# intel/neural-speed

Hardware: AMD Instinct MI355X
Metric: decode_tokens_per_sec (higher is better)
Workload: dtype f16; 1 GPU; Llama-2-7B Q4_0 (BesTLA int4 sym g32 bf16-scale) batch=1 decode GEMM chain: 32 layers x {QKV, WO, FFN gate/up, FFN down} + lm_head; parallelism=tp1, launch=hipGraph replay, weights_bytes_per_gpu=3716481024

## Files before the change

neural-speed_amd/csrc/ns_gemv.hip:

```cpp
#include <hip/hip_runtime.h>

#include <algorithm>
#include <atomic>
#include <cmath>
#include <cstddef>
#include <cstdlib>
#include <cstring>
#include <type_traits>
#include <utility>

#include "../../include/ns_bestla.h"
#include "ns_common.h"
#include "ns_route.h"
#include "ns_dev.h"

namespace ns {

#ifndef NS_GV_PF
#define NS_GV_PF 4
#endif
constexpr int kGvPF = NS_GV_PF;
constexpr int kGvMaxRows = 16;
constexpr size_t kGvMaxALds = 64 * 1024;
constexpr size_t kGvMaxLds = 160 * 1024;
// ... 66 lines not shown
  GemvRope rope;
  F4Lut lut;
  F8Consts f8;
#ifdef NS_TRACE
  unsigned long long* trace;
#endif
};
using KArgs = const __attribute__((address_space(4))) GemvParams*;
__device__ __forceinline__ KArgs late_args() {
  uint64_t v = reinterpret_cast<uint64_t>(__builtin_amdgcn_kernarg_segment_ptr());
  asm volatile("" : "+s"(v));
  return reinterpret_cast<KArgs>(v);
}

#ifdef NS_TRACE
#define NS_GSTAMP(i)                                                                                     \
  do {                                                                                                   \
    __builtin_amdgcn_sched_barrier(0);                                                                   \
    if ((threadIdx.x & 63) == 0 && blockIdx.x < 4096)                                                     \
      p.trace[(size_t(blockIdx.x) * 16 + (threadIdx.x >> 6)) * 8 + (i)] = wall_clock64();                 \
    __builtin_amdgcn_sched_barrier(0);                                                                   \
  } while (0)
#else
#define NS_GSTAMP(i)
#endif

template <int N>
__device__ __forceinline__ void wait_vmcnt() {
  asm volatile("s_waitcnt vmcnt(%0)" ::"n"(N) : "memory");
}

enum GemvMode { GV_PLAIN = 0, GV_DUAL = 1, GV_MSEG = 2 };
constexpr int kGvA32Regs = 8;
template <int KIND, int SPS, int SK, bool ASYM, int MODE, int XV, bool PL = false>
__global__ __launch_bounds__(1024) void gemv_kernel(const GemvParams p) {
  constexpr bool EXT = XV == 1, MOE = XV == 4, I8Q = XV == 5, A32 = XV == 2 || MOE || I8Q, I8S = XV == 3 || I8Q;
  static_assert(!PL || ((KIND == WK_INT4 || KIND == WK_INT8) && !I8S && !MOE), "native planes: integer formats, fp16 numerics");
  static_assert(!I8S || KIND == WK_INT4 || KIND == WK_INT8, "integer weights only");
  constexpr uint32_t AEL = I8S ? 1u : 2u;
  constexpr bool DUAL = MODE == GV_DUAL, MSEG = MODE == GV_MSEG;
  constexpr int NJ = kind_is_8bit(KIND) ? 2 : 4;
  constexpr int KSTEP = NJ * 32;
  constexpr int NQ = DUAL ? 2 : 1;
  constexpr int PF = kGvPF;
  static_assert(PF % NQ == 0, "ring slots alternate between the two matrices");
  constexpr int SBYTES = SPS * (SK == SK_F32 ? 4 : 2);
  using Corr = CorrRaw<SPS, SK, ASYM>;
  extern __shared__ __attribute__((aligned(16))) unsigned char smem[];
  _Float16* a_lds = reinterpret_cast<_Float16*>(smem);
  NS_GSTAMP(0);

  {
    asm volatile("" ::"s"(p.wbase0), "s"(p.a), "s"(p.ks), "s"(p.qstride), "s"(p.nw_log2), "s"(p.s_off0), "s"(p.sstride),
                 "s"(p.srows), "s"(p.srow_mul), "s"(p.srow_shift), "s"(p.m), "s"(p.k), "s"(p.lda), "s"(p.row_stride),
                 "s"(p.ring_off), "s"(p.ring_stride));
    if constexpr (DUAL) asm volatile("" ::"s"(p.wbase1), "s"(p.s_off1));
    if constexpr (MSEG)
      asm volatile("" ::"s"(p.tb1), "s"(p.tb2), "s"(p.mat[0].wbase), "s"(p.mat[1].wbase), "s"(p.mat[2].wbase), "s"(p.mat[0].s_off),
                   "s"(p.mat[1].s_off), "s"(p.mat[2].s_off));
    if constexpr (ASYM) asm volatile("" ::"s"(p.z_off0), "s"(p.z_off1), "s"(p.zstride));
    if constexpr (PL) asm volatile("" ::"s"(p.pl_bits), "s"(p.pl_lanes));
  }
  const int tid = threadIdx.x;
  const uint32_t w = __builtin_amdgcn_readfirstlane(tid >> 6);
  const int l = tid & 63;
  const int nn = l & 15, g = l >> 4;
  const uint32_t NW = 1u << p.nw_log2;
  const uint32_t ks = p.ks;
  const uint32_t T = blockIdx.x;
// ... 20 lines not shown
    const int e = *p.moe_id;
    if (e < 0 || e >= p.moe_n) {
      const KArgs cz = late_args();
      const int colz = int(T) * 16 + nn;
      if (w == 0 && g == 0 && colz < cz->mat[0].n) {
        float v = 0.f;
        const float dv = cz->d ? cz->d[colz] : 0.f;
        switch (cz->epilogue) {
          case 1: v = v + dv; break;
          case 2: v = v * dv; break;
          case 3: v = epi_gelu(v + dv); break;
          case 4: v = epi_gelu(v); break;
          case 5: v = epi_silu(v); break;
          default: break;
        }
        cz->mat[0].c[colz] = v;
        if (cz->mat[0].c16) cz->mat[0].c16[colz] = (_Float16)v;
      }
      return;
    }
    rw[0] = make_rsrc(p.moe_table[e].codes, 0x80000000u);
    so[0] = p.s_off0;
    zo[0] = p.z_off0;
  } else {
    rw[0] = make_rsrc(p.wbase0, 0x80000000u);
    so[0] = p.s_off0;
    zo[0] = p.z_off0;
  }
  const uint32_t tile_q = tl * ks * p.qstride;
  const uint32_t tile_c = tl * p.srows;
  const uint32_t voff_q = l * 16, voff_s = nn * SBYTES, voff_z = nn * SPS;
  const I4Consts i4c = {0x000f000fu, 0x00f000f0u, 0x64006400u};

  constexpr uint32_t SLOT = 1024u + 16u * SBYTES + (ASYM ? 16u * SPS : 0u);
  constexpr int OPS = ASYM ? 3 : 2;
  static_assert(OPS * PF + kGvMaxRows * 2 <= 63, "vmcnt is a 6-bit counter (ring + the carried norm's pieces)");
  const LdsPtr ring = (LdsPtr)(smem) + p.ring_off + w * p.ring_stride;
  const uint32_t ring_lane = uint32_t(reinterpret_cast<uintptr_t>(ring)) + uint32_t(l) * 16u;
  const uint32_t ring_corr = uint32_t(reinterpret_cast<uintptr_t>(ring)) + 1024u + uint32_t(nn) * SBYTES;

  auto issue = [&](auto slot_c, uint32_t s) {
    constexpr int slot = decltype(slot_c)::value;
    constexpr int q = slot % NQ;
#if defined(__HIP_DEVICE_COMPILE__)
    const uint32_t crow = tile_c + ((s * p.srow_mul) >> p.srow_shift);
    const LdsPtr dst = ring + slot * SLOT;
    if (!PL || uint32_t(l) < p.pl_lanes)
      __builtin_amdgcn_raw_ptr_buffer_load_lds(rw[q], reinterpret_cast<__attribute__((address_space(3))) void*>(dst), 16, voff_q,
                                               tile_q + s * p.qstride, 0, 2);
    if (l < SBYTES)
      __builtin_amdgcn_raw_ptr_buffer_load_lds(rw[q], reinterpret_cast<__attribute__((address_space(3))) void*>(dst + 1024), 16,
                                               voff_q, so[q] + crow * p.sstride, 0, 2);
    if constexpr (ASYM) {
      if (l < SPS)
        __builtin_amdgcn_raw_ptr_buffer_load_lds(rw[q], reinterpret_cast<__attribute__((address_space(3))) void*>(dst + 1024 + 16 * SBYTES),
                                                 16, voff_q, zo[q] + crow * p.zstride, 0, 2);
    }
#endif
  };
  auto wait_records = [&](uint32_t younger) {
    if (younger == uint32_t(PF - 1)) {
      wait_vmcnt<OPS * (PF - 1)>();
      return;
    }
    [&]<int... K>(std::integer_sequence<int, K...>) {
      (void)((younger == uint32_t(K) ? (wait_vmcnt<OPS * K>(), true) : false) || ...);
    }(std::make_integer_sequence<int, PF + 1>{});
  };

#define NS_FOR_SLOTS(BODY)                                        \
  {                                                               \
    [&]<int... I>(std::integer_sequence<int, I...>) {             \
      (([&] { constexpr int i = I; std::integral_constant<int, I> ic; (void)i; (void)ic; BODY }()), ...); \
    }(std::make_integer_sequence<int, PF>{});                     \
  }

  const int rows = min(p.m, kGvMaxRows);
  floatx4 areg[A32 ? kGvA32Regs : 1];
  if constexpr (A32) {
    const uint64_t abase = reinterpret_cast<uint64_t>(p.a);
    const uint4v ra_words = {uint32_t(abase), uint32_t(abase >> 32) & 0xffffu,
                             uint32_t(rows - 1) * uint32_t(p.lda) * 4u + uint32_t(p.k) * 4u, 0x00020000u};
    const uint32_t row_bytes = ks * uint32_t(KSTEP) * 4u;
    const uint32_t pieces = (row_bytes + 1023u) >> 10;
    const uint32_t total = uint32_t(rows) * pieces;
    uint32_t r = 0, c = w;
#pragma unroll
    for (int i = 0; i < kGvA32Regs; i++) {
      const uint32_t u = w + (uint32_t(i) << p.nw_log2);
      areg[i] = floatx4{0.f, 0.f, 0.f, 0.f};
      if (u < total) {
// ... 10 lines not shown
  } else {
    const Rsrc ra = make_rsrc(p.a, uint32_t(rows - 1) * uint32_t(p.lda) * AEL + uint32_t(p.k) * AEL);
    const uint32_t row_bytes = ks * uint32_t(KSTEP) * AEL;
    const uint32_t pieces = (row_bytes + 1023u) >> 10;
    const uint32_t total = uint32_t(rows) * pieces;
    const LdsPtr al = (LdsPtr)(smem);
    for (uint32_t u = w; u < total; u += NW) {
      uint32_t r = 0, c = u;
      if (rows > 1) {
        r = u / pieces;
        c = u - r * pieces;
      }
      const uint32_t left = row_bytes - (c << 10);
#if defined(__HIP_DEVICE_COMPILE__)
      if (uint32_t(l) * 16u < left)
        __builtin_amdgcn_raw_ptr_buffer_load_lds(ra, reinterpret_cast<__attribute__((address_space(3))) void*>(al + r * p.row_stride * 2u + (c << 10)),
                                                 16, voff_q, r * uint32_t(p.lda) * AEL + (c << 10), 0, 0);
#endif
    }
    if constexpr (I8S) {
      const Rsrc rc = make_rsrc(p.i8_corr, p.i8_span);
      for (uint32_t u = w; u < ((p.i8_span + 1023u) >> 10); u += NW) {
#if defined(__HIP_DEVICE_COMPILE__)
        __builtin_amdgcn_raw_ptr_buffer_load_lds(rc, reinterpret_cast<__attribute__((address_space(3))) void*>(al + p.ssq_off + (u << 10)), 16,
                                                 voff_q, u << 10, 0, 0);
#endif
      }
    }
  }
  __builtin_amdgcn_sched_barrier(0);

  const uint32_t first = w;
  const uint32_t nst = first < ks ? (ks - first + NW - 1) >> p.nw_log2 : 0u;
  NS_FOR_SLOTS({ if (uint32_t(i / NQ) < nst) issue(ic, first + ((i / NQ) << p.nw_log2)); })
  __builtin_amdgcn_sched_barrier(0);
  NS_GSTAMP(1);

  const float* in_ssq = nullptr;
  uint32_t in_parts = 0, ssq_off = 0;
  if constexpr (EXT) {
    const KArgs mid = late_args();
    in_ssq = mid->in_ssq;
    in_parts = mid->in_parts;
    ssq_off = mid->ssq_off;
  }
  if (EXT && in_ssq && w == 0) {
    const uint32_t in_stride = late_args()->in_stride;
    const uint32_t spieces = (in_parts * 4u + 1023u) >> 10;
    const Rsrc rs = make_rsrc(in_ssq, (uint32_t(rows - 1) * in_stride + in_parts) * 4u);
    const LdsPtr al = (LdsPtr)(smem);
    for (uint32_t u = 0; u < uint32_t(rows) * spieces; u++) {
      const uint32_t r = u / spieces, c = u - r * spieces;
      const uint32_t left = in_parts * 4u - (c << 10);
#if defined(__HIP_DEVICE_COMPILE__)
      if (uint32_t(l) * 16u < left)
        __builtin_amdgcn_raw_ptr_buffer_load_lds(rs, reinterpret_cast<__attribute__((address_space(3))) void*>(al + ssq_off + (u << 10)),
                                                 16, voff_q, r * in_stride * 4u + (c << 10), 0, 0);
#endif
    }
  }
  __builtin_amdgcn_sched_barrier(0);

  wait_records(min(nst * uint32_t(NQ), uint32_t(PF)));
  if constexpr (A32) {
#pragma unroll
    for (int i = 0; i < kGvA32Regs; i++) asm volatile("" : "+v"(areg[i]));
    const uint32_t row_bytes = ks * uint32_t(KSTEP) * 4u;
    const uint32_t pieces = (row_bytes + 1023u) >> 10;
    const uint32_t total = uint32_t(rows) * pieces;
    uint32_t r = 0, c = w;
    if constexpr (I8Q) {
      const uint32_t lds0q = uint32_t(reinterpret_cast<uintptr_t>((LdsPtr)(smem)));
      const uint32_t lpb = 1u << (p.i8_bshift - 2u);
      const uint32_t k_bytes = uint32_t(p.k) * 4u;
#pragma unroll
      for (int i = 0; i < kGvA32Regs; i++) {
        const uint32_t u = w + (uint32_t(i) << p.nw_log2);
        if (u < total) {
          while (c >= pieces) c -= pieces, r++;
          const floatx4 v = areg[i];
          float maxval = 1.17549435e-38f , minval = 0.f;
#pragma unroll
          for (int e = 0; e < 4; e++) {
            maxval = v[e] > maxval ? v[e] : maxval;
            minval = v[e] < minval ? v[e] : minval;
          }
          auto dpp = [](float x, auto ctrl) {
            return __builtin_bit_cast(float, __builtin_amdgcn_update_dpp(0, __builtin_bit_cast(int, x), decltype(ctrl)::value, 0xf, 0xf, false));
          };
          auto combine = [&](float om, float on) {
            maxval = om > maxval ? om : maxval;
            minval = on < minval ? on : minval;
          };
          combine(dpp(maxval, std::integral_constant<int, 0xB1>{}), dpp(minval, std::integral_constant<int, 0xB1>{}));
          combine(dpp(maxval, std::integral_constant<int, 0x4E>{}), dpp(minval, std::integral_constant<int, 0x4E>{}));
          combine(dpp(maxval, std::integral_constant<int, 0x141>{}), dpp(minval, std::integral_constant<int, 0x141>{}));
// ... 25 lines not shown
        }
      }
    } else {
#pragma unroll
    for (int i = 0; i < kGvA32Regs; i++) {
      const uint32_t u = w + (uint32_t(i) << p.nw_log2);
      if (u < total) {
        while (c >= pieces) c -= pieces, r++;
        const half2_t lo = half2_t{(_Float16)areg[i][0], (_Float16)areg[i][1]};
        const half2_t hi = half2_t{(_Float16)areg[i][2], (_Float16)areg[i][3]};
        const uint32_t dst = uint32_t(reinterpret_cast<uintptr_t>((LdsPtr)(smem))) + r * p.row_stride * 2u + (c << 9) + uint32_t(l) * 8u;
        if ((c << 10) + uint32_t(l) * 16u < row_bytes)
          asm volatile("ds_write_b64 %0, %1" ::"v"(dst), "v"((uint64_t(as_u32(hi)) << 32) | as_u32(lo)) : "memory");
        c += NW;
      }
    }
    }
    asm volatile("s_waitcnt lgkmcnt(0)" ::: "memory");
  }
  asm volatile("s_barrier" ::: "memory");
  NS_GSTAMP(2);

  const uint32_t aoff = uint32_t(min(nn, rows - 1)) * p.row_stride + 8 * g;
  floatx4 acc[NQ];
#pragma unroll
  for (int q = 0; q < NQ; q++) acc[q] = floatx4{0.f, 0.f, 0.f, 0.f};

  float accr[NQ][4];
#pragma unroll
  for (int q = 0; q < NQ; q++)
#pragma unroll
    for (int r = 0; r < 4; r++) accr[q][r] = 0.f;
  const uint32_t i8_rsb = p.row_stride * 2u;
  auto compute = [&](auto slot_c, uint32_t s) {
    constexpr int slot = decltype(slot_c)::value;
    constexpr int q = slot % NQ;
#if defined(NS_GV_ABL) && NS_GV_ABL == 1
    (void)s;
    return;
#endif
    if constexpr (I8S) {
      Corr cr;
      {
        typedef __attribute__((address_space(3))) const uint32_t* L32;
        const uint32_t ca = ring_corr + uint32_t(slot) * SLOT;
        if constexpr (SBYTES == 2) {
          cr.s[0] = *reinterpret_cast<__attribute__((address_space(3))) const uint16_t*>(ca);
        } else {
#pragma unroll
          for (int t = 0; t < Corr::NW32; t++) cr.s[t] = reinterpret_cast<L32>(ca)[t];
        }
        if constexpr (ASYM) {
          const uint32_t za = uint32_t(reinterpret_cast<uintptr_t>(ring)) + uint32_t(slot) * SLOT + 1024u + 16u * SBYTES + uint32_t(nn) * SPS;
          if constexpr (SPS == 4)
            cr.z[0] = *reinterpret_cast<L32>(za);
          else if constexpr (SPS == 2)
            cr.z[0] = *reinterpret_cast<__attribute__((address_space(3))) const uint16_t*>(za);
          else
            cr.z[0] = *reinterpret_cast<__attribute__((address_space(3))) const uint8_t*>(za);
        }
      }
      float sc[4], zp[4];
      corr_decode<SPS, SK, ASYM, NJ>(cr, sc, zp);
      const uint4v qvv = *reinterpret_cast<const __attribute__((address_space(3))) uint4v*>(ring_lane + uint32_t(slot) * SLOT);
      const uint32_t xw[4] = {qvv.x, qvv.y, qvv.z, qvv.w};
      constexpr int BIAS = KIND == WK_INT4 ? 8 : 128;
      const uint32_t lds0 = uint32_t(reinterpret_cast<uintptr_t>((LdsPtr)(smem)));
      const uint32_t kbase = s * uint32_t(KSTEP);
      const uint32_t i8_sbase = lds0 + p.ssq_off;
// ... 27 lines not shown
                "ds_read_b32 %8, %17\n\tds_read_b32 %9, %18\n\tds_read_b32 %10, %19\n\tds_read_b32 %11, %20\n\ts_waitcnt lgkmcnt(0)"
                : "=&v"(av[0]), "=&v"(av[1]), "=&v"(av[2]), "=&v"(av[3]), "=&v"(zau[0]), "=&v"(zau[1]), "=&v"(zau[2]), "=&v"(zau[3]),
                  "=&v"(asu[0]), "=&v"(asu[1]), "=&v"(asu[2]), "=&v"(asu[3])
                : "v"(aaddr), "v"(zrow + kb[0]), "v"(zrow + kb[1]), "v"(zrow + kb[2]), "v"(zrow + kb[3]), "v"(srow + kb[0] * 4u),
                  "v"(srow + kb[1] * 4u), "v"(srow + kb[2] * 4u), "v"(srow + kb[3] * 4u)
                : "memory");
          } else {
            asm volatile(
                "ds_read_b64 %0, %6\n\tds_read_b64 %1, %6 offset:32\n\tds_read_u8 %2, %7\n\tds_read_u8 %3, %8\n\t"
                "ds_read_b32 %4, %9\n\tds_read_b32 %5, %10\n\ts_waitcnt lgkmcnt(0)"
                : "=&v"(av[0]), "=&v"(av[1]), "=&v"(zau[0]), "=&v"(zau[1]), "=&v"(asu[0]), "=&v"(asu[1])
                : "v"(aaddr), "v"(zrow + kb[0]), "v"(zrow + kb[1]), "v"(srow + kb[0] * 4u), "v"(srow + kb[1] * 4u)
                : "memory");
          }
#pragma unroll
          for (int j = 0; j < NJ; j++) {
            if (kbase + 32u * uint32_t(j) < uint32_t(p.k)) {
              const uint32_t avx = uint32_t(av[j]), avy = uint32_t(av[j] >> 32);
              const int za = int(zau[j]);
              const int dot = int(__builtin_amdgcn_udot4(avx, u0[j], __builtin_amdgcn_udot4(avy, u1[j], 0u, false), false));
              const int sa = int(__builtin_amdgcn_udot4(avx, 0x01010101u, __builtin_amdgcn_udot4(avy, 0x01010101u, 0u, false), false));
              const int isum = dot - zbq[j] * sa - za * su[j] + 8 * za * zbq[j];
              accr[q][r] += float(isum) * (__builtin_bit_cast(float, asu[j]) * sc[j]);
            }
          }
        }
      }
      return;
    }
    const _Float16* abase = a_lds + s * KSTEP + aoff;
    Corr cr;
    {
      typedef __attribute__((address_space(3))) const uint32_t* L32;
      const uint32_t ca = ring_corr + uint32_t(slot) * SLOT;
      if constexpr (SBYTES == 2) {
        cr.s[0] = *reinterpret_cast<__attribute__((address_space(3))) const uint16_t*>(ca);
      } else {
#pragma unroll
        for (int t = 0; t < Corr::NW32; t++) cr.s[t] = reinterpret_cast<L32>(ca)[t];
      }
      if constexpr (ASYM) {
        const uint32_t za = uint32_t(reinterpret_cast<uintptr_t>(ring)) + uint32_t(slot) * SLOT + 1024u + 16u * SBYTES + uint32_t(nn) * SPS;
        if constexpr (SPS == 4)
          cr.z[0] = *reinterpret_cast<L32>(za);
        else if constexpr (SPS == 2)
          cr.z[0] = *reinterpret_cast<__attribute__((address_space(3))) const uint16_t*>(za);
        else
          cr.z[0] = *reinterpret_cast<__attribute__((address_space(3))) const uint8_t*>(za);
      }
    }
    float sc[4], zp[4];
    corr_decode<SPS, SK, ASYM, NJ>(cr, sc, zp);
    uint32_t xw[4];
    if constexpr (!PL) {
      const uint4v qvv = *reinterpret_cast<const __attribute__((address_space(3))) uint4v*>(ring_lane + uint32_t(slot) * SLOT);
      xw[0] = qvv.x, xw[1] = qvv.y, xw[2] = qvv.z, xw[3] = qvv.w;
    } else {
      typedef const __attribute__((address_space(3))) uint32_t* L32;
      typedef const __attribute__((address_space(3))) uint16_t* L16;
      typedef uint32_t uint2v __attribute__((ext_vector_type(2)));
      const uint32_t rec = uint32_t(reinterpret_cast<uintptr_t>(ring)) + uint32_t(slot) * SLOT;
      const uint32_t bits = p.pl_bits;
      if constexpr (KIND == WK_INT4) {
        uint32_t a0 = 0, a1 = 0, cw = 0;
        if (bits >= 2) {
          const uint2v av = *reinterpret_cast<const __attribute__((address_space(3))) uint2v*>(rec + 8u * uint32_t(l));
          a0 = av.x, a1 = av.y;
// ... 28 lines not shown
        bq[j] = cvt_i4x8(xw[j], i4c, half2_t{zl, zl}, half2_t{zh, zh});
      } else if constexpr (KIND == WK_INT8) {
        if constexpr (PL) {
          const _Float16 zo8 = (_Float16)(-1024.f - full - zp[j]);
          bq[j] = cvt_u8x8(xw[2 * j], xw[2 * j + 1], half2_t{zo8, zo8});
        } else {
          const _Float16 zo8 = (_Float16)(-1152.f - zp[j]);
          bq[j] = cvt_i8x8(xw[2 * j], xw[2 * j + 1], half2_t{zo8, zo8});
        }
      } else if constexpr (KIND == WK_F8) {
        bq[j] = cvt_f8x8(xw[2 * j], xw[2 * j + 1], p.f8);
      } else {
        bq[j] = cvt_f4x8(xw[j], p.lut);
      }
    }
    floatx4 dd[NJ];
#pragma unroll
    for (int j = 0; j < NJ; j++) {
      const half8_t afrag = *reinterpret_cast<const half8_t*>(abase + 32 * j);
      dd[j] = __builtin_amdgcn_mfma_f32_16x16x32_f16(afrag, bq[j], floatx4{0.f, 0.f, 0.f, 0.f}, 0, 0, 0);
    }
#pragma unroll
    for (int j = 0; j < NJ; j++) acc[q] += dd[j] * sc[j];
  };

  constexpr int SPR = PF / NQ;
  const uint32_t rounds = (nst + SPR - 1) / SPR;
  const uint32_t nitems = nst * NQ;
  for (uint32_t r = 0; r < rounds; r++) {
    NS_FOR_SLOTS({
      const uint32_t ord = r * SPR + i / NQ;
      if (ord < nst) {
        const uint32_t t = r * PF + i;
        wait_records(min(nitems - t - 1, uint32_t(PF - 1)));
        compute(ic, first + (ord << p.nw_log2));
        __builtin_amdgcn_sched_barrier(0);
        if (ord + SPR < nst) issue(ic, first + ((ord + SPR) << p.nw_log2));
        __builtin_amdgcn_sched_barrier(0);
      }
    })
  }
  NS_GSTAMP(4);

  if constexpr (I8S) {
#pragma unroll
    for (int q = 0; q < NQ; q++) {
      float t[4];
#pragma unroll
      for (int r = 0; r < 4; r++) {
        float v = accr[q][r];
        v += __shfl_xor(v, 16, 64);
        v += __shfl_xor(v, 32, 64);
        t[r] = v;
      }
      acc[q] = g == 0 ? floatx4{t[0], t[1], t[2], t[3]} : floatx4{0.f, 0.f, 0.f, 0.f};
    }
  }
  floatx4* red = reinterpret_cast<floatx4*>(smem + p.ring_off);
  const uint32_t kRedWave = p.ring_stride / 16;
#pragma unroll
  for (int q = 0; q < NQ; q++) red[w * kRedWave + q * 64 + l] = acc[q];
  const KArgs cold = late_args();
  const auto* mp = &cold->mat[MSEG ? sg : 0];
  const int ncols = mp->n;
  float* cbase = mp->c;
  _Float16* c16 = mp->c16;
  const int ldc = cold->ldc, ldd = cold->ldd, epi = cold->epilogue;
  const float* dptr = cold->d;
  float* c2 = cold->c2;
// ... 108 lines not shown
            case 5: v = epi_silu(v); break;
            default: break;
          }
        }
        cbase[size_t(row) * ldc + col] = v;
        if (c16) c16[size_t(row) * ldc + col] = (_Float16)(v * gam);
        if constexpr (EXT) {
          if (ogamma && fabsf(v * gam) > 65504.f && cold->out_ovf) __hip_atomic_store(cold->out_ovf, 1u, __ATOMIC_RELAXED, __HIP_MEMORY_SCOPE_SYSTEM);
        }
      }
      if (EXT && ossq) {
        float t = ok ? v * v : 0.f;
        t += __shfl_xor(t, 1, 64);
        t += __shfl_xor(t, 2, 64);
        t += __shfl_xor(t, 4, 64);
        t += __shfl_xor(t, 8, 64);
        if (nn == 0 && row < p.m) ossq[size_t(row) * ostride + tl] = t;
      }
    }
  }
#undef NS_FOR_SLOTS
  NS_GSTAMP(6);
#ifdef NS_TRACE
  if ((threadIdx.x & 63) == 0 && blockIdx.x < 4096)
    p.trace[(size_t(blockIdx.x) * 16 + (threadIdx.x >> 6)) * 8 + 7] =
        (uint64_t(__builtin_amdgcn_s_getreg((31 << 11) | 20)) << 32) | uint32_t(__builtin_amdgcn_s_getreg((31 << 11) | 4));
#endif
}

constexpr int kGvModeA32 = 0x100;
constexpr int kGvModeI8 = 0x200;
constexpr int kGvModeMoe = 0x400;
constexpr int kGvModePlanes = 0x800;
template <int KIND, int SPS, int SK, bool ASYM>
static hipError_t launch_gemv_planes(const GemvParams& p, int mode, int grid, int nw, size_t lds, hipStream_t st) {
  if constexpr ((KIND == WK_INT4 || KIND == WK_INT8) && SK != SK_F16) {
    const dim3 g(grid), b(nw * 64);
    const bool ext = p.in_ssq || p.out_gamma || p.out_ssq || p.rope.on;
    const bool a32 = (mode & kGvModeA32) != 0;
    mode &= 3;
#define NS_GVP(MODEV, EXTV)                                                                                                  \
  {                                                                                                                         \
    auto k = gemv_kernel<KIND, SPS, SK, ASYM, MODEV, EXTV, true>;                                                            \
    static const hipError_t attr =                                                                                          \
        hipFuncSetAttribute(reinterpret_cast<const void*>(k), hipFuncAttributeMaxDynamicSharedMemorySize, int(kGvMaxLds));   \
    if (attr != hipSuccess && lds > 64 * 1024) return attr;                                                                 \
    hipLaunchKernelGGL(k, g, b, lds, st, p);                                                                                \
  }
#define NS_GVP_M(MODEV)                                                              \
  {                                                                                 \
    if (ext) NS_GVP(MODEV, 1) else if (a32) NS_GVP(MODEV, 2) else NS_GVP(MODEV, 0)   \
  }
    if (mode == GV_DUAL)
      NS_GVP_M(GV_DUAL)
    else if (mode == GV_MSEG)
      NS_GVP_M(GV_MSEG)
    else
      NS_GVP_M(GV_PLAIN)
#undef NS_GVP_M
#undef NS_GVP
    return hipGetLastError();
  } else {
    return hipErrorNotSupported;
  }
}
template <int KIND, int SPS, int SK, bool ASYM>
static hipError_t launch_gemv_k(const GemvParams& p, int mode, int grid, int nw, size_t lds, hipStream_t st) {
  if (mode & kGvModePlanes) return launch_gemv_planes<KIND, SPS, SK, ASYM>(p, mode & ~kGvModePlanes, grid, nw, lds, st);
  const dim3 g(grid), b(nw * 64);
  const bool ext = p.in_ssq || p.out_gamma || p.out_ssq || p.rope.on;
  const bool a32 = (mode & kGvModeA32) != 0;
  const bool i8s = (mode & kGvModeI8) != 0;
  const bool moe = (mode & kGvModeMoe) != 0;
  mode &= ~(kGvModeA32 | kGvModeI8 | kGvModeMoe);
  if (moe) {
    if constexpr (KIND == WK_F8) return hipErrorNotSupported;
    if (mode != GV_PLAIN) return hipErrorNotSupported;
  }
  if constexpr (KIND != WK_INT4 && KIND != WK_INT8)
    if (i8s) return hipErrorNotSupported;
#define NS_GV_LAUNCH(MODEV)                                                                                     \
  {                                                                                                             \
    if (moe) NS_GV_LAUNCH_MOE(MODEV) else if (ext) NS_GV_LAUNCH_E(MODEV, 1) else if (i8s && a32) NS_GV_LAUNCH_I8Q(MODEV) else if (a32) NS_GV_LAUNCH_E(MODEV, 2) else if (i8s) NS_GV_LAUNCH_I8(MODEV)    \
    else NS_GV_LAUNCH_E(MODEV, 0)                                                                               \
  }
#define NS_GV_LAUNCH_MOE(MODEV)                                                                                  \
  {                                                                                                             \
    if constexpr (KIND != WK_F8 && MODEV == GV_PLAIN) NS_GV_LAUNCH_E(GV_PLAIN, 4)                               \
  }
#define NS_GV_LAUNCH_I8Q(MODEV)                                                                                  \
  {                                                                                                             \
    if constexpr (KIND == WK_INT4 || KIND == WK_INT8) NS_GV_LAUNCH_E(MODEV, 5)                                  \
  }
#define NS_GV_LAUNCH_I8(MODEV)                                                                                   \
  {                                                                                                             \
    if constexpr (KIND == WK_INT4 || KIND == WK_INT8) NS_GV_LAUNCH_E(MODEV, 3)                                  \
  }
#define NS_GV_LAUNCH_E(MODEV, EXTV)                                                                             \
  {                                                                                                             \
    auto k = gemv_kernel<KIND, SPS, SK, ASYM, MODEV, EXTV>;                                                      \
    static const hipError_t attr =                                                                              \
        hipFuncSetAttribute(reinterpret_cast<const void*>(k), hipFuncAttributeMaxDynamicSharedMemorySize, int(kGvMaxLds)); \
    if (attr != hipSuccess && lds > 64 * 1024) return attr;                                                     \
    hipLaunchKernelGGL(k, g, b, lds, st, p);                                                                    \
  }
  if (mode == GV_DUAL)
    NS_GV_LAUNCH(GV_DUAL)
  else if (mode == GV_MSEG)
    NS_GV_LAUNCH(GV_MSEG)
  else
    NS_GV_LAUNCH(GV_PLAIN)
#undef NS_GV_LAUNCH
#undef NS_GV_LAUNCH_E
#undef NS_GV_LAUNCH_I8
#undef NS_GV_LAUNCH_I8Q
#undef NS_GV_LAUNCH_MOE
  return hipGetLastError();
}
template <int KIND, int SPS, int SK>
static hipError_t launch_gemv_a(const GemvParams& p, bool asym, int mode, int grid, int nw, size_t lds,
                                hipStream_t st) {
  if constexpr (KIND == WK_F4 || KIND == WK_F8) {
    (void)asym;
    return launch_gemv_k<KIND, SPS, SK, false>(p, mode, grid, nw, lds, st);
  } else {
    if (asym) return launch_gemv_k<KIND, SPS, SK, true>(p, mode, grid, nw, lds, st);
    return launch_gemv_k<KIND, SPS, SK, false>(p, mode, grid, nw, lds, st);
  }
}
template <int KIND, int SPS>
static hipError_t launch_gemv_s(const GemvParams& p, uint32_t scale_dt, bool asym, int mode, int grid, int nw,
                                size_t lds, hipStream_t st) {
  if (scale_dt == DT_F32) return launch_gemv_a<KIND, SPS, SK_F32>(p, asym, mode, grid, nw, lds, st);
  if (scale_dt == DT_F16) return launch_gemv_a<KIND, SPS, SK_F16>(p, asym, mode, grid, nw, lds, st);
  return launch_gemv_a<KIND, SPS, SK_BF16>(p, asym, mode, grid, nw, lds, st);
}

#ifdef NS_TRACE
unsigned long long* trace_buffer();
#endif

static std::atomic<int> g_gemv_mode{-1};
void set_gemv_mode(int mode) { g_gemv_mode.store(mode); }
static int gemv_mode() {
  int m = g_gemv_mode.load();
  if (m < 0) {
// ... 2 lines not shown
    g_gemv_mode.store(m);
  }
  return m;
}

static std::atomic<int> g_decode_waves{0};
void set_decode_waves(int nw) { g_decode_waves.store(nw); }
int decode_waves(int grid, int ks, bool dual) {
  int nw = (grid <= 320 && ks >= 32 && ks <= 48 && !dual) ? 16 : 8;
  if (dual) {
    nw = grid * 4 >= 1300 ? 4 : 8;
  } else {
    const int target_waves = 2560;
    while (nw > 2 && grid * (nw / 2) >= target_waves) nw /= 2;
  }
  static const int env_nw0 = getenv("NS_GV_NW") ? atoi(getenv("NS_GV_NW")) : 0;
  const int forced = g_decode_waves.load();
  const int env_nw = forced ? forced : env_nw0;
  if (env_nw == 2 || env_nw == 4 || env_nw == 8 || (env_nw == 16 && !dual)) nw = env_nw;
  while (nw > 1 && nw > ks) nw /= 2;
  return nw;
}

static std::atomic<int> g_gemv_planes{-1};
void set_gemv_planes(int on) { g_gemv_planes.store(on != 0); }
static bool gemv_planes() {
  int v = g_gemv_planes.load();
  if (v < 0) {
    const char* e = getenv("NS_GEMV_PLANES");
    v = e ? atoi(e) != 0 : 1;
    g_gemv_planes.store(v);
  }
  return v != 0;
}

hipError_t launch_gemv(const SmallMArgs& a, hipStream_t st) {
  if (gemv_mode() == 0 || a.m < 1 || a.m > kGvMaxRows) return hipErrorNotSupported;
  const int nmat = a.nseg;
  bool planes = gemv_planes() && !a.i8 && !a.moe;
  for (int i = 0; i < nmat; i++)
    planes = planes && a.seg[i].w->native && a.seg[i].w->native->scale_dt != DT_F16 && a.seg[i].w->native->pl_bits == a.seg[0].w->native->pl_bits;
  auto pick = [&](const ns_weight* w) { return planes ? static_cast<const ns_weight*>(w->native) : w; };
  const ns_weight* w0 = pick(a.seg[0].w);
  GemvParams p;
  memset(&p, 0, sizeof(p));
  uint32_t tiles = 0;
  uint32_t tbeg[3] = {0, 0xffffffffu, 0xffffffffu};
  const uint8_t* wb[3] = {nullptr, nullptr, nullptr};
  uint32_t soff[3] = {0, 0, 0}, zoff[3] = {0, 0, 0};
  for (int i = 0; i < nmat; i++) {
    const ns_weight* w = pick(a.seg[i].w);
    if (!w->single_span || w->alloc_bytes >= (size_t(1) << 31)) return hipErrorNotSupported;
    wb[i] = reinterpret_cast<const uint8_t*>(w->codes);
    soff[i] = uint32_t(reinterpret_cast<const uint8_t*>(w->scales) - wb[i]);
    zoff[i] = w->zps ? uint32_t(reinterpret_cast<const uint8_t*>(w->zps) - wb[i]) : 0u;
    tbeg[i] = a.dual ? 0u : tiles;
    if (!a.dual || i == 0) tiles += uint32_t(w->ntiles);
    p.mat[i] = GemvMat{wb[i], soff[i], zoff[i], tbeg[i], w->n, a.seg[i].c, static_cast<_Float16*>(a.seg[i].c16)};
  }
  const bool mseg = !a.dual && nmat > 1;
  const int mode = a.dual ? GV_DUAL : (mseg ? GV_MSEG : GV_PLAIN);
  p.wbase0 = wb[0];
  p.wbase1 = wb[1];
  p.s_off0 = soff[0], p.s_off1 = soff[1], p.z_off0 = zoff[0], p.z_off1 = zoff[1];
  p.tb1 = mseg ? tbeg[1] : 0xffffffffu;
  p.tb2 = (mseg && nmat > 2) ? tbeg[2] : 0xffffffffu;
// ... 52 lines not shown
    if (k.out_ssq || k.out_gamma) {
      if (a.dual || nmat != 1 || (k.out_ssq && k.out_stride < w0->ntiles)) return hipErrorInvalidValue;
      p.out_gamma = k.out_gamma, p.out_ssq = k.out_ssq, p.out_stride = uint32_t(k.out_stride);
      p.out_ovf = k.out_gamma ? kvm_overflow_word() : nullptr;
    }
  }
  if (a.rope) {
    const ns_qkv_rope& r = *a.rope;
    if (mode != GV_MSEG || nmat != 3 || r.mode != 0 || r.head_size < 2 || (r.head_size & 1) || r.n_dims != r.head_size ||
        !r.kcache16 || !r.vcache16 || !r.cos_sin || r.n_past < 0 || p.mat[0].n != r.heads * r.head_size ||
        p.mat[1].n != r.heads_kv * r.head_size || p.mat[2].n != r.heads_kv * r.head_size)
      return hipErrorInvalidValue;
    p.rope.kc = static_cast<_Float16*>(r.kcache16), p.rope.vc = static_cast<_Float16*>(r.vcache16);
    p.rope.c_sl = r.cache_step_sl, p.rope.c_head = r.cache_step_head;
    p.rope.head_size = r.head_size, p.rope.n_past = r.n_past;
    p.rope.cos_sin = reinterpret_cast<const float2*>(r.cos_sin);
    p.rope.on = 1;
    if (a.rope_route) {
      const QkvRopeRoute& q = *a.rope_route;
      if (rows != 1) return hipErrorInvalidValue;
      p.rope.kmove = q.kmove, p.rope.kd_pos = q.kd_pos;
      p.rope.k32 = q.k32, p.rope.v32 = q.v32;
      p.rope.k32_head = q.k32_head, p.rope.k32_dim = q.k32_dim, p.rope.k32_tok = q.k32_tok;
      p.rope.v32_head = q.v32_head, p.rope.v32_dim = q.v32_dim, p.rope.v32_tok = q.v32_tok;
      p.rope.ovf = q.overflow;
    }
  }
  if (uint64_t(rows) * uint64_t(a.lda) * 4 >= (uint64_t(1) << 30)) return hipErrorNotSupported;

  const int grid = int(tiles);
  const int nq = a.dual ? 2 : 1;
  const uint32_t sbytes = uint32_t(w0->sps) * (w0->scale_dt == DT_F32 ? 4u : 2u);
  const uint32_t slot = 1024u + 16u * sbytes + (w0->asym ? 16u * uint32_t(w0->sps) : 0u);
  auto ring_bytes = [&](int waves) {
    const uint32_t items = ((ks + uint32_t(waves) - 1) / uint32_t(waves)) * uint32_t(nq);
    const size_t b = size_t(std::min<uint32_t>(items, uint32_t(kGvPF))) * slot;
    return std::max<size_t>((b + 15) & ~size_t(15), size_t(nq) * 1024);
  };
  int nw = decode_waves(grid, int(ks), a.dual);
  {
    while (nw > 1 && ((a_bytes + 15) & ~size_t(15)) + ssq_bytes + size_t(nw) * ring_bytes(nw) > kGvMaxLds) nw /= 2;
  }
  uint32_t nw_log2 = 0;
  while ((1 << nw_log2) < nw) nw_log2++;
  if (a32 && uint64_t(rows) * ((uint64_t(ks) * uint32_t(kstep) * 4u + 1023u) >> 10) > uint64_t(nw) * kGvA32Regs) {
    if (i8q) return a.i8->quantized ? hipErrorNotSupported : hipErrorNotReady;
    return hipErrorNotSupported;
  }

  p.ks = ks;
  p.qstride = w0->qstride;
  p.nw_log2 = nw_log2;
  p.sstride = w0->sstride;
  p.zstride = w0->zstride;
  p.srows = uint32_t(w0->srows);
  {
    int mul, shift;
    if (!srow_params(w0, &mul, &shift)) return hipErrorNotSupported;
    p.srow_mul = uint32_t(mul), p.srow_shift = uint32_t(shift);
  }
  p.m = a.m;
  p.k = w0->k;
  p.lda = i8q ? a.i8->lda32 : i8s ? a.i8->ldq : a.lda;
  p.row_stride = row_stride;
  p.ssq_off = uint32_t((a_bytes + 15) & ~size_t(15));
  p.ring_off = p.ssq_off + uint32_t(ssq_bytes);
  p.c2 = a.c2;
  p.d = a.d;
  p.ldc = a.ldc;
  p.ldd = a.ldd;
  p.epilogue = a.epilogue;
  if (w0->kind == WK_F4) f4_lut_planes(w0->lut, &p.lut);
  p.f8 = f8_consts(w0->qtype);
#ifdef NS_TRACE
  p.trace = trace_buffer();
#endif
  p.ring_stride = uint32_t(ring_bytes(nw));
  const size_t lds = size_t(p.ring_off) + size_t(nw) * p.ring_stride;
  if (lds > kGvMaxLds) return hipErrorNotSupported;
  if (moe) {
    p.moe_table = static_cast<const MoeExpertRow*>(a.moe->table);
    p.moe_id = a.moe->id;
    p.moe_n = a.moe->n_as;
  }
  p.pl_bits = planes ? uint32_t(w0->pl_bits) : 0u;
  p.pl_lanes = planes ? w0->code_rec / 16u : 64u;
  const int mode_x = mode | (a32 && !moe ? kGvModeA32 : 0) | (i8s ? kGvModeI8 : 0) | (moe ? kGvModeMoe : 0) | (planes ? kGvModePlanes : 0);

#define NS_DISPATCH(KIND)                                                                       \
  switch (w0->sps) {                                                                            \
    case 4: return launch_gemv_s<KIND, 4>(p, w0->scale_dt, w0->asym, mode_x, grid, nw, lds, st);  \
    case 2: return launch_gemv_s<KIND, 2>(p, w0->scale_dt, w0->asym, mode_x, grid, nw, lds, st);  \
    default: return launch_gemv_s<KIND, 1>(p, w0->scale_dt, w0->asym, mode_x, grid, nw, lds, st); \
  }
  if (w0->kind == WK_INT4) {
    NS_DISPATCH(WK_INT4)
  } else if (w0->kind == WK_INT8) {
    if (w0->sps == 2) return launch_gemv_s<WK_INT8, 2>(p, w0->scale_dt, w0->asym, mode_x, grid, nw, lds, st);
    return launch_gemv_s<WK_INT8, 1>(p, w0->scale_dt, w0->asym, mode_x, grid, nw, lds, st);
  } else if (w0->kind == WK_F8) {
    if (w0->sps == 2) return launch_gemv_a<WK_F8, 2, SK_F32>(p, false, mode_x, grid, nw, lds, st);
    return launch_gemv_a<WK_F8, 1, SK_F32>(p, false, mode_x, grid, nw, lds, st);
  } else {
    NS_DISPATCH(WK_F4)
  }
#undef NS_DISPATCH
}

void touch_gemv_module() {
  hipFuncAttributes fa;
  (void)hipFuncGetAttributes(&fa, reinterpret_cast<const void*>(gemv_kernel<WK_INT4, 4, SK_BF16, false, GV_PLAIN, 0>));
  (void)hipGetLastError();
}
}
```

Baseline: 939.7 tokens/s.

## Gather bf16 group scales for four k-steps in one batched LDS load

For the int4 sym g32 bf16-scale path, the per-slot 16-lane scale buffer load is dropped. Each wave instead issues one gathered load that fetches the scales for four upcoming k-steps into a small double-buffered LDS region, and the vmcnt accounting is rewritten to match. This cuts the number of tiny global loads and vmcnt slots per k-step, and shrinks each ring slot. The cost is extra waits, an lgkmcnt drain before each gather, and more complex, error-prone counter bookkeeping. A host check keeps the path off unless alignment, bounds and LDS-occupancy conditions hold, and an environment variable can disable it.

```diff
diff --git a/neural-speed_amd/csrc/ns_gemv.hip b/neural-speed_amd/csrc/ns_gemv.hip
--- a/neural-speed_amd/csrc/ns_gemv.hip
+++ b/neural-speed_amd/csrc/ns_gemv.hip
@@ -122,9 +122,11 @@
 
 enum GemvMode { GV_PLAIN = 0, GV_DUAL = 1, GV_MSEG = 2 };
 constexpr int kGvA32Regs = 8;
-template <int KIND, int SPS, int SK, bool ASYM, int MODE, int XV, bool PL = false>
+template <int KIND, int SPS, int SK, bool ASYM, int MODE, int XV, bool PL = false, bool SG = false>
 __global__ __launch_bounds__(1024) void gemv_kernel(const GemvParams p) {
   constexpr bool EXT = XV == 1, MOE = XV == 4, I8Q = XV == 5, A32 = XV == 2 || MOE || I8Q, I8S = XV == 3 || I8Q;
+  static_assert(!SG || (KIND == WK_INT4 && SPS == 4 && SK == SK_BF16 && !ASYM && !PL && MODE != GV_DUAL && (XV == 0 || XV == 1) && kGvPF == 4),
+                "scale gather: the flagship's instantiations only");
   static_assert(!PL || ((KIND == WK_INT4 || KIND == WK_INT8) && !I8S && !MOE), "native planes: integer formats, fp16 numerics");
   static_assert(!I8S || KIND == WK_INT4 || KIND == WK_INT8, "integer weights only");
   constexpr uint32_t AEL = I8S ? 1u : 2u;
@@ -211,9 +213,10 @@
   const uint32_t voff_q = l * 16, voff_s = nn * SBYTES, voff_z = nn * SPS;
   const I4Consts i4c = {0x000f000fu, 0x00f000f0u, 0x64006400u};
 
-  constexpr uint32_t SLOT = 1024u + 16u * SBYTES + (ASYM ? 16u * SPS : 0u);
-  constexpr int OPS = ASYM ? 3 : 2;
-  static_assert(OPS * PF + kGvMaxRows * 2 <= 63, "vmcnt is a 6-bit counter (ring + the carried norm's pieces)");
+  constexpr uint32_t SLOT = SG ? 1024u : 1024u + 16u * SBYTES + (ASYM ? 16u * SPS : 0u);
+  constexpr int OPS = SG ? 1 : (ASYM ? 3 : 2);
+  constexpr int GIF = SG ? 2 : 0;
+  static_assert(OPS * PF + GIF + kGvMaxRows * 2 <= 63, "vmcnt is a 6-bit counter (ring + gathers + the carried norm's pieces)");
   const LdsPtr ring = (LdsPtr)(smem) + p.ring_off + w * p.ring_stride;
   const uint32_t ring_lane = uint32_t(reinterpret_cast<uintptr_t>(ring)) + uint32_t(l) * 16u;
   const uint32_t ring_corr = uint32_t(reinterpret_cast<uintptr_t>(ring)) + 1024u + uint32_t(nn) * SBYTES;
@@ -222,11 +225,12 @@
     constexpr int slot = decltype(slot_c)::value;
     constexpr int q = slot % NQ;
 #if defined(__HIP_DEVICE_COMPILE__)
-    const uint32_t crow = tile_c + ((s * p.srow_mul) >> p.srow_shift);
+    const uint32_t crow = SG ? 0u : tile_c + ((s * p.srow_mul) >> p.srow_shift);
     const LdsPtr dst = ring + slot * SLOT;
     if (!PL || uint32_t(l) < p.pl_lanes)
       __builtin_amdgcn_raw_ptr_buffer_load_lds(rw[q], reinterpret_cast<__attribute__((address_space(3))) void*>(dst), 16, voff_q,
                                                tile_q + s * p.qstride, 0, 2);
+    if constexpr (SG) return;
     if (l < SBYTES)
       __builtin_amdgcn_raw_ptr_buffer_load_lds(rw[q], reinterpret_cast<__attribute__((address_space(3))) void*>(dst + 1024), 16,
                                                voff_q, so[q] + crow * p.sstride, 0, 2);
@@ -236,6 +240,11 @@
                                                  16, voff_q, zo[q] + crow * p.zstride, 0, 2);
     }
 #endif
+  };
+  auto wait_requests = [&](uint32_t n) {
+    [&]<int... K>(std::integer_sequence<int, K...>) {
+      (void)((n == uint32_t(K) ? (wait_vmcnt<K>(), true) : false) || ...);
+    }(std::integer_sequence<int, 4, 3, 2, 1, 0, 5, 6>{});
   };
   auto wait_records = [&](uint32_t younger) {
     if (younger == uint32_t(PF - 1)) {
@@ -312,6 +321,24 @@
 
   const uint32_t first = w;
   const uint32_t nst = first < ks ? (ks - first + NW - 1) >> p.nw_log2 : 0u;
+  const LdsPtr sring = ring + p.ring_stride - 1024u;
+  const uint32_t sring_corr = uint32_t(reinterpret_cast<uintptr_t>(sring)) + uint32_t(nn) * SBYTES;
+  const uint32_t voff_g = SG ? ((uint32_t(l) >> 3) << p.nw_log2) * p.sstride + (uint32_t(l) & 7u) * 16u : 0u;
+  (void)sring_corr;
+  (void)voff_g;
+  auto gather = [&](uint32_t j) {
+#if defined(__HIP_DEVICE_COMPILE__)
+    if (uint32_t(l) < 32u && 4u * j + (uint32_t(l) >> 3) < nst)
+      __builtin_amdgcn_raw_ptr_buffer_load_lds(rw[0], reinterpret_cast<__attribute__((address_space(3))) void*>(sring + (j & 1u) * 512u), 16,
+                                               voff_g, so[0] + (tile_c + first + ((4u * j) << p.nw_log2)) * p.sstride, 0, 2);
+#endif
+  };
+  (void)gather;
+  (void)wait_requests;
+  if constexpr (SG) {
+    if (nst > 0u) gather(0u);
+    if (nst > 4u) gather(1u);
+  }
   NS_FOR_SLOTS({ if (uint32_t(i / NQ) < nst) issue(ic, first + ((i / NQ) << p.nw_log2)); })
   __builtin_amdgcn_sched_barrier(0);
   NS_GSTAMP(1);
@@ -341,7 +368,8 @@
   }
   __builtin_amdgcn_sched_barrier(0);
 
-  wait_records(min(nst * uint32_t(NQ), uint32_t(PF)));
+  if constexpr (SG) wait_requests(min(nst, uint32_t(PF)) + (nst > 0u ? 1u : 0u) + (nst > 4u ? 1u : 0u));
+  else wait_records(min(nst * uint32_t(NQ), uint32_t(PF)));
   if constexpr (A32) {
 #pragma unroll
     for (int i = 0; i < kGvA32Regs; i++) asm volatile("" : "+v"(areg[i]));
@@ -433,9 +461,10 @@
 #pragma unroll
     for (int r = 0; r < 4; r++) accr[q][r] = 0.f;
   const uint32_t i8_rsb = p.row_stride * 2u;
-  auto compute = [&](auto slot_c, uint32_t s) {
+  auto compute = [&](auto slot_c, uint32_t s, uint32_t ord) {
     constexpr int slot = decltype(slot_c)::value;
     constexpr int q = slot % NQ;
+    (void)ord;
 #if defined(NS_GV_ABL) && NS_GV_ABL == 1
     (void)s;
     return;
@@ -529,7 +558,7 @@
     Corr cr;
     {
       typedef __attribute__((address_space(3))) const uint32_t* L32;
-      const uint32_t ca = ring_corr + uint32_t(slot) * SLOT;
+      const uint32_t ca = SG ? sring_corr + (ord & 7u) * 128u : ring_corr + uint32_t(slot) * SLOT;
       if constexpr (SBYTES == 2) {
         cr.s[0] = *reinterpret_cast<__attribute__((address_space(3))) const uint16_t*>(ca);
       } else {
@@ -624,9 +653,20 @@
       const uint32_t ord = r * SPR + i / NQ;
       if (ord < nst) {
         const uint32_t t = r * PF + i;
-        wait_records(min(nitems - t - 1, uint32_t(PF - 1)));
-        compute(ic, first + (ord << p.nw_log2));
+        if constexpr (SG) {
+          const uint32_t gathers = (i != PF - 1 && r > 0u && 4u * r + 4u < nst) ? 1u : 0u;
+          wait_requests(min(nst - t - 1, uint32_t(PF - 1)) + gathers);
+        } else {
+          wait_records(min(nitems - t - 1, uint32_t(PF - 1)));
+        }
+        compute(ic, first + (ord << p.nw_log2), ord);
         __builtin_amdgcn_sched_barrier(0);
+        if constexpr (SG) {
+          if (i == PF - 1 && 4u * r + 8u < nst) {
+            asm volatile("s_waitcnt lgkmcnt(0)" ::: "memory");
+            gather(r + 2u);
+          }
+        }
         if (ord + SPR < nst) issue(ic, first + ((ord + SPR) << p.nw_log2));
         __builtin_amdgcn_sched_barrier(0);
       }
@@ -801,6 +841,9 @@
 constexpr int kGvModeI8 = 0x200;
 constexpr int kGvModeMoe = 0x400;
 constexpr int kGvModePlanes = 0x800;
+constexpr int kGvModeSG = 0x1000;
+template <int KIND, int SPS, int SK, bool ASYM, int MODE, int XV>
+constexpr bool kGvHasSG = KIND == WK_INT4 && SPS == 4 && SK == SK_BF16 && !ASYM && MODE != GV_DUAL && (XV == 0 || XV == 1) && kGvPF == 4;
 template <int KIND, int SPS, int SK, bool ASYM>
 static hipError_t launch_gemv_planes(const GemvParams& p, int mode, int grid, int nw, size_t lds, hipStream_t st) {
   if constexpr ((KIND == WK_INT4 || KIND == WK_INT8) && SK != SK_F16) {
@@ -841,7 +884,8 @@
   const bool a32 = (mode & kGvModeA32) != 0;
   const bool i8s = (mode & kGvModeI8) != 0;
   const bool moe = (mode & kGvModeMoe) != 0;
-  mode &= ~(kGvModeA32 | kGvModeI8 | kGvModeMoe);
+  const bool sg = (mode & kGvModeSG) != 0;
+  mode &= ~(kGvModeA32 | kGvModeI8 | kGvModeMoe | kGvModeSG);
   if (moe) {
     if constexpr (KIND == WK_F8) return hipErrorNotSupported;
     if (mode != GV_PLAIN) return hipErrorNotSupported;
@@ -867,7 +911,14 @@
   }
 #define NS_GV_LAUNCH_E(MODEV, EXTV)                                                                             \
   {                                                                                                             \
-    auto k = gemv_kernel<KIND, SPS, SK, ASYM, MODEV, EXTV>;                                                      \
+    if (sg) {                                                                                                   \
+      if constexpr (kGvHasSG<KIND, SPS, SK, ASYM, MODEV, EXTV>) NS_GV_LAUNCH_K(MODEV, EXTV, true)               \
+      else return hipErrorInvalidValue;            \
+    } else NS_GV_LAUNCH_K(MODEV, EXTV, false)                                                                   \
+  }
+#define NS_GV_LAUNCH_K(MODEV, EXTV, SGV)                                                                        \
+  {                                                                                                             \
+    auto k = gemv_kernel<KIND, SPS, SK, ASYM, MODEV, EXTV, false, SGV>;                                          \
     static const hipError_t attr =                                                                              \
         hipFuncSetAttribute(reinterpret_cast<const void*>(k), hipFuncAttributeMaxDynamicSharedMemorySize, int(kGvMaxLds)); \
     if (attr != hipSuccess && lds > 64 * 1024) return attr;                                                     \
@@ -881,6 +932,7 @@
     NS_GV_LAUNCH(GV_PLAIN)
 #undef NS_GV_LAUNCH
 #undef NS_GV_LAUNCH_E
+#undef NS_GV_LAUNCH_K
 #undef NS_GV_LAUNCH_I8
 #undef NS_GV_LAUNCH_I8Q
 #undef NS_GV_LAUNCH_MOE
@@ -949,6 +1001,23 @@
     g_gemv_planes.store(v);
   }
   return v != 0;
+}
+
+static bool device_lds_and_cus(int dev, size_t* lds, int* cus) {
+  constexpr int kMaxDev = 64;
+  static std::atomic<int> s_lds[kMaxDev], s_cus[kMaxDev];
+  if (dev < 0 || dev >= kMaxDev) return false;
+  int l = s_lds[dev].load(), c = s_cus[dev].load();
+  if (l <= 0 || c <= 0) {
+    if (hipDeviceGetAttribute(&l, hipDeviceAttributeMaxSharedMemoryPerMultiprocessor, dev) != hipSuccess ||
+        hipDeviceGetAttribute(&c, hipDeviceAttributeMultiprocessorCount, dev) != hipSuccess || l <= 0 || c <= 0) {
+      (void)hipGetLastError();
+      return false;
+    }
+    s_lds[dev].store(l), s_cus[dev].store(c);
+  }
+  *lds = size_t(l), *cus = c;
+  return true;
 }
 
 hipError_t launch_gemv(const SmallMArgs& a, hipStream_t st) {
@@ -1067,9 +1136,10 @@
   const int nq = a.dual ? 2 : 1;
   const uint32_t sbytes = uint32_t(w0->sps) * (w0->scale_dt == DT_F32 ? 4u : 2u);
   const uint32_t slot = 1024u + 16u * sbytes + (w0->asym ? 16u * uint32_t(w0->sps) : 0u);
-  auto ring_bytes = [&](int waves) {
+  auto ring_bytes = [&](int waves, bool gathered = false) {
     const uint32_t items = ((ks + uint32_t(waves) - 1) / uint32_t(waves)) * uint32_t(nq);
-    const size_t b = size_t(std::min<uint32_t>(items, uint32_t(kGvPF))) * slot;
+    const size_t b = gathered ? size_t(std::min<uint32_t>(items, uint32_t(kGvPF))) * 1024 + 1024
+                              : size_t(std::min<uint32_t>(items, uint32_t(kGvPF))) * slot;
     return std::max<size_t>((b + 15) & ~size_t(15), size_t(nq) * 1024);
   };
   int nw = decode_waves(grid, int(ks), a.dual);
@@ -1111,8 +1181,35 @@
   p.trace = trace_buffer();
 #endif
   p.ring_stride = uint32_t(ring_bytes(nw));
-  const size_t lds = size_t(p.ring_off) + size_t(nw) * p.ring_stride;
+  size_t lds = size_t(p.ring_off) + size_t(nw) * p.ring_stride;
   if (lds > kGvMaxLds) return hipErrorNotSupported;
+  bool sg = kGvPF == 4 && w0->kind == WK_INT4 && w0->sps == 4 && w0->scale_dt == DT_BF16 && !w0->asym &&
+            !planes && !a.dual && !i8s && !moe && !a32 && p.srow_mul == 1 && p.srow_shift == 0 && (p.sstride & 15) == 0;
+  if (sg) {
+    const char* e = getenv("NS_GV_SCALE_GATHER");
+    sg = !(e && atoi(e) == 0);
+  }
+  for (int i = 0; sg && i < nmat; i++) {
+    const ns_weight* w = pick(a.seg[i].w);
+    sg = (reinterpret_cast<uintptr_t>(wb[i]) & 15) == 0 && (soff[i] & 15) == 0 && w->sstride == p.sstride && w->sps == 4 && !w->asym &&
+         uint32_t(w->srows) == p.srows && uint32_t(w->ksteps) == ks && w->ntiles > 0 && p.srows >= ks &&
+         uint64_t(soff[i]) + (uint64_t(w->ntiles - 1) * p.srows + ks - 1) * p.sstride + 128 <= uint64_t(w->alloc_bytes);
+  }
+  if (sg) {
+    const size_t ring_sg = ring_bytes(nw, true);
+    const size_t lds_sg = size_t(p.ring_off) + size_t(nw) * ring_sg;
+    size_t cu_lds = 0;
+    int cus = 0;
+    sg = lds_sg <= kGvMaxLds && device_lds_and_cus(w0->device, &cu_lds, &cus);
+    if (sg) {
+      const size_t before = cu_lds / lds, after = cu_lds / lds_sg, need = (size_t(grid) + size_t(cus) - 1) / size_t(cus);
+      sg = after >= std::min(before, need);
+    }
+    if (sg) {
+      p.ring_stride = uint32_t(ring_sg);
+      lds = lds_sg;
+    }
+  }
   if (moe) {
     p.moe_table = static_cast<const MoeExpertRow*>(a.moe->table);
     p.moe_id = a.moe->id;
@@ -1120,7 +1217,8 @@
   }
   p.pl_bits = planes ? uint32_t(w0->pl_bits) : 0u;
   p.pl_lanes = planes ? w0->code_rec / 16u : 64u;
-  const int mode_x = mode | (a32 && !moe ? kGvModeA32 : 0) | (i8s ? kGvModeI8 : 0) | (moe ? kGvModeMoe : 0) | (planes ? kGvModePlanes : 0);
+  const int mode_x = mode | (a32 && !moe ? kGvModeA32 : 0) | (i8s ? kGvModeI8 : 0) | (moe ? kGvModeMoe : 0) | (planes ? kGvModePlanes : 0) |
+                     (sg ? kGvModeSG : 0);
 
 #define NS_DISPATCH(KIND)                                                                       \
   switch (w0->sps) {                                                                            \
```

Result: no change. 935.0 tokens/s (-0.5%).
